# DeepBlender/DeepDenoiser

Hardware: AMD Instinct MI355X
Metric: train tiles/sec (128x128x32ch U-Net KPCN) (higher is better)
Workload: dtype bf16; 1 GPU; BASELINE config 2: U-Net [64,96,128]x4 + 5x5 KernelPrediction + 3-scale MultiScalePrediction, 32-channel render-pass stack, 128x128 tiles, full training step (fwd+SMAPE loss+bwd+Adam); global_batch=128, parallelism=dp1, hipgraph=True, inputs=resident in HBM

## Files before the change

deepdenoiser_amd/_lib.py:

```python

import ctypes as C
import os

_HERE = os.path.dirname(os.path.abspath(__file__))
LIB_PATH = os.environ.get("DD_LIB", os.path.join(_HERE, "libdd_hip.so"))

DD_F32, DD_BF16, DD_F16 = 0, 1, 2
IN_RELU, OUT_RELU, ACCUM, PIXSHUF, GATHER2X2 = 1, 2, 4, 8, 16
MAX_FEATURES, MAX_COMBINED = 32, 8
METRIC_SOURCES = MAX_FEATURES + MAX_COMBINED + 1
HISTOGRAM_DIFFERENCE, HISTOGRAM_VARIATION_DIFFERENCE, HISTOGRAM_MASKED_DIFFERENCE = 0, 1, 2
HISTOGRAM_VALUES_SCRATCH_BYTES = 20480
PREVIEW_SOURCE, PREVIEW_PREDICTION, PREVIEW_TARGET, PREVIEW_DIFFERENCE = 1, 2, 4, 8
PREVIEW_MAX_IMAGES, PREVIEW_THRESHOLDS = 16, 255
NONFINITE_MAX_PLANES = 32
QUALITY_MAX_PAIRS, QUALITY_TILE = 32, 32
GRAD_CHUNK, GRAD_PARTIAL_BYTES = 4096, 24


def histogram_stats_offset(nb):
    return (nb + 1) // 2 * 8


def histogram_record_bytes(nb):
    return histogram_stats_offset(nb) + 48


SYMBOLS = (
    "dd_version", "dd_last_error", "dd_pack_weights", "dd_pack_weights_batched", "dd_conv_igemm", "dd_conv_wgrad", "dd_colsum", "dd_colsum_segments",
    "dd_maxpool_fwd", "dd_maxpool_bwd", "dd_avgpool", "dd_prepare_feature", "dd_gather_input",
    "dd_kpcn_fwd", "dd_kpcn_bwd", "dd_kpcn_hidden_fwd", "dd_kpcn_hidden_bwd", "dd_compose_pack", "dd_compose_blend_fwd", "dd_compose_blend_bwd",
    "dd_compose_unpack_bwd", "dd_invert_std_fwd", "dd_invert_std_bwd", "dd_loss_head", "dd_adam_step",
    "dd_stitch", "dd_recombine", "dd_probe_tr16", "dd_masked_add", "dd_zero_stuff", "dd_zero_unstuff", "dd_convert_channels",
    "dd_augment", "dd_loss_mask_sums", "dd_crc32c", "dd_extract_tiles", "dd_compose_net_fwd", "dd_compose_net_bwd",
    "dd_kpcn_head_fwd", "dd_kpcn_head_bwd", "dd_kpcn_head_bwd_multi", "dd_assemble_input", "dd_assemble_input_frames", "dd_conv3x3_bwd", "dd_conv3x3_bwd_multi", "dd_convt2x2_fwd", "dd_convt2x2_bwd", "dd_convt_bwd_wide_count", "dd_conv3x3_ks",
    "dd_conv_pw_count", "dd_wgrad_pw_count", "dd_conv_route_count", "dd_space_to_depth2", "dd_convt3_wgrad", "dd_compose_stream_plan", "dd_compose_bwd_scratch_bytes",
    "dd_loss_msssim_scratch_bytes", "dd_loss_msssim_fwd", "dd_loss_msssim_bwd", "dd_loss_msssim_values",
    "dd_loss_metrics_scratch_bytes", "dd_loss_metrics", "dd_loss_head_path_count",
    "dd_loss_head_dscale", "dd_loss_msssim_bwd_dscale", "dd_grads_nonfinite", "dd_adam_step_scaled", "dd_scaler_update",
    "dd_histogram_values", "dd_loss_histograms_scratch_bytes", "dd_loss_histograms", "dd_loss_previews",
    "dd_nonfinite_scan", "dd_nonfinite_repair", "dd_frame_quality_scratch_bytes", "dd_frame_quality", "dd_stitch_blend",
    "dd_grad_norms", "dd_adam_step_clipped", "dd_adam_step_scaled_clipped", "dd_sample_tiles",
)


ROUTES = ("igemm_resident", "igemm_streamed", "igemm_ws", "rw_6_2", "rw12", "rw12_mask", "rw12_res", "rw8_kc2", "rw8_kc4", "rw8_kc4_mask", "pw",
          "ks", "ks_pw_taps", "wgrad_dma", "wgrad_reg", "wgrad_pw", "wgrad_stacked")


def route_counts():
    lib = load()
    return {name: lib.dd_conv_route_count(r) for r, name in enumerate(ROUTES)}


SUBROUTES = ("rw8_k32",)


def subroute_counts():
    lib = load()
    return {name: lib.dd_conv_route_count(len(ROUTES) + r) for r, name in enumerate(SUBROUTES)}


class ConvT3WgradArgs(C.Structure):
    _fields_ = [("s", C.c_void_p), ("lds", C.c_int), ("cout", C.c_int), ("cp", C.c_int),
                ("x", C.c_void_p), ("ldx", C.c_int), ("cin", C.c_int),
                ("dk", C.c_void_p),
                ("B", C.c_int), ("H", C.c_int), ("W", C.c_int), ("dtype", C.c_int)]


class ConvArgs(C.Structure):
    _fields_ = [("x", C.c_void_p), ("ldx", C.c_int), ("cin", C.c_int),
                ("wp", C.c_void_p), ("k_pad", C.c_int), ("n_pad", C.c_int),
                ("bias", C.c_void_p), ("nbias", C.c_int),
                ("res", C.c_void_p), ("ldres", C.c_int),
                ("mask", C.c_void_p), ("ldmask", C.c_int),
                ("y", C.c_void_p), ("ldy", C.c_int), ("n", C.c_int),
                ("B", C.c_int), ("H", C.c_int), ("W", C.c_int),
                ("taps", C.c_int), ("flags", C.c_int), ("dtype", C.c_int)]


class WgradArgs(C.Structure):
    _fields_ = [("p", C.c_void_p), ("ldp", C.c_int), ("m", C.c_int),
                ("q", C.c_void_p), ("ldq", C.c_int), ("n", C.c_int),
                ("out", C.c_void_p), ("bias_out", C.c_void_p), ("bias_mode", C.c_int),
                ("B", C.c_int), ("H", C.c_int), ("W", C.c_int),
                ("taps", C.c_int), ("flags", C.c_int), ("dtype", C.c_int), ("ksplit", C.c_int),
                ("stack_blocks", C.c_int), ("stack_width", C.c_int), ("stack_m0", C.c_int),
                ("stack_out", C.c_void_p * 8), ("stack_bias", C.c_void_p * 8)]
# ... 205 lines not shown
    if _lib is not None:
        return _lib
    import torch
    if not os.path.exists(LIB_PATH):
        raise RuntimeError("libdd_hip.so is not built (%s missing): run `python -m deepdenoiser_amd.build`. "
                           "There is no CPU/PyTorch fallback for the hot path." % LIB_PATH)
    lib = C.CDLL(LIB_PATH)
    missing = [s for s in SYMBOLS if not hasattr(lib, s)]
    if missing:
        raise RuntimeError("libdd_hip.so lacks symbols %s: rebuild it" % missing)
    lib.dd_version.restype = C.c_char_p
    lib.dd_last_error.restype = C.c_char_p
    _check_source_hash(lib)
    for s in SYMBOLS[2:]:
        getattr(lib, s).restype = C.c_int
    vp, i, l, f = C.c_void_p, C.c_int, C.c_long, C.c_float
    lib.dd_pack_weights.argtypes = [vp, vp, i, i, i, i, i, i, l, l, l, i, vp]
    lib.dd_pack_weights_batched.argtypes = [vp, i, i, vp]
    lib.dd_conv_igemm.argtypes = [C.POINTER(ConvArgs), vp]
    lib.dd_conv_wgrad.argtypes = [C.POINTER(WgradArgs), vp]
    lib.dd_conv3x3_bwd.argtypes = [C.POINTER(ConvBwdArgs), vp]
    lib.dd_conv3x3_bwd_multi.argtypes = [C.POINTER(ConvBwdArgs), i, vp]
    lib.dd_convt2x2_fwd.argtypes = [C.POINTER(ConvTArgs), vp]
    lib.dd_convt2x2_bwd.argtypes = [C.POINTER(ConvTArgs), vp]
    lib.dd_conv3x3_ks.argtypes = [C.POINTER(ConvKsArgs), vp]
    lib.dd_space_to_depth2.argtypes = [vp, i, vp, i, i, i, i, i, i, i, vp]
    lib.dd_convt3_wgrad.argtypes = [C.POINTER(ConvT3WgradArgs), vp]
    lib.dd_conv_pw_count.argtypes = []
    lib.dd_conv_pw_count.restype = C.c_long
    lib.dd_wgrad_pw_count.argtypes = []
    lib.dd_wgrad_pw_count.restype = C.c_long
    lib.dd_convt_bwd_wide_count.argtypes = []
    lib.dd_convt_bwd_wide_count.restype = C.c_long
    lib.dd_conv_route_count.argtypes = [i]
    lib.dd_conv_route_count.restype = C.c_long
    lib.dd_colsum.argtypes = [vp, i, i, l, vp, i, vp]
    lib.dd_colsum_segments.argtypes = [vp, i, i, l, i, vp, i, vp, i, vp]
    lib.dd_maxpool_fwd.argtypes = [vp, i, vp, i, vp, i, i, i, i, i, i, i, i, vp]
    lib.dd_maxpool_bwd.argtypes = [vp, i, vp, vp, i, vp, i, i, i, i, i, i, i, i, i, vp]
    lib.dd_avgpool.argtypes = [vp, i, vp, i, i, i, i, i, i, vp]
    lib.dd_prepare_feature.argtypes = [vp, i, vp, i, C.POINTER(FeatureParams), i, i, i, vp]
    lib.dd_gather_input.argtypes = [vp, i, i, vp, i, i, i, i, i, i, vp]
    lib.dd_kpcn_fwd.argtypes = [vp, i, vp, i, vp, i, i, i, i, i, i, vp]
    lib.dd_kpcn_bwd.argtypes = [vp, i, vp, i, vp, i, vp, i, i, i, i, i, i, i, vp]
    lib.dd_kpcn_hidden_fwd.argtypes = [vp, i, vp, i, i, vp, i, vp, vp, i, i, i, i, i, i, vp]
    lib.dd_kpcn_hidden_bwd.argtypes = [vp, i, vp, i, i, vp, i, vp, vp, i, vp, i, i, i, i, i, i, i, vp]
    lib.dd_compose_pack.argtypes = [vp, i, vp, i, vp, i, i, i, i, i, i, vp]
    lib.dd_compose_blend_fwd.argtypes = [vp, i, vp, i, vp, i, vp, i, i, i, i, i, vp]
    lib.dd_compose_blend_bwd.argtypes = [vp, i, vp, i, vp, i, vp, i, vp, i, i, vp, i, vp, i, i, i, i, i, i, vp]
    lib.dd_compose_unpack_bwd.argtypes = [vp, i, vp, i, vp, i, i, i, i, i, vp]
    lib.dd_invert_std_fwd.argtypes = [vp, vp, l, i, f, f, vp]
    lib.dd_invert_std_bwd.argtypes = [vp, vp, vp, l, i, f, f, vp]
    lib.dd_loss_head.argtypes = [C.POINTER(LossDesc), i, i, i, vp, f, vp]
    lib.dd_loss_head_path_count.argtypes = [i]
    lib.dd_loss_head_path_count.restype = C.c_long
    lib.dd_loss_msssim_scratch_bytes.argtypes = [i, i, i, i]
    lib.dd_loss_msssim_scratch_bytes.restype = C.c_long
    lib.dd_loss_msssim_fwd.argtypes = [C.POINTER(MsSsimDesc), i, i, i, vp, vp, vp]
    lib.dd_loss_msssim_bwd.argtypes = [C.POINTER(MsSsimDesc), i, i, i, vp, f, vp]
    lib.dd_loss_msssim_values.argtypes = [C.POINTER(MsSsimDesc), i, i, i, vp, vp, vp]
    lib.dd_loss_metrics_scratch_bytes.argtypes = [i, i, i]
    lib.dd_loss_metrics_scratch_bytes.restype = C.c_long
    lib.dd_loss_metrics.argtypes = [C.POINTER(LossDesc), i, i, i, vp, vp, vp]
    lib.dd_histogram_values.argtypes = [vp, l, vp, i, vp, vp, vp]
    lib.dd_loss_histograms_scratch_bytes.argtypes = [i, i, i, i]
    lib.dd_loss_histograms_scratch_bytes.restype = C.c_long
# ... 48 lines not shown
```

deepdenoiser_amd/csrc/dd_conv_bwd.hip:

```cpp
#include "dd_common.h"

#ifndef CBW_DF_RING
#define CBW_DF_RING 2
#endif
#ifndef CBW_REUSE
#define CBW_REUSE 1
#endif
#ifndef BW_DMA_SPAN
#define BW_DMA_SPAN 8
#endif
namespace {

struct BwdP {
  const void* dy; const void* x; const void* wd; void* dx; float* dw; float* db;
  int lddy, ldx, lddx;
  int cout, cin, coutv, cinv;
  int n_pad, k_pad;
  int B, H, W, tiles_x, tiles_y;
  int nblk, nblk_co, ksplit;
  int co_base;
  int use_mask, accumulate;
};

typedef __attribute__((address_space(3))) s16x4_t* lds_tr_ptr;
// ... 4 lines not shown

__device__ __forceinline__ void bw_dma_1k(const void* gptr, unsigned lds_addr) {
  asm volatile("s_mov_b32 m0, %1\n\ts_nop 0\n\tglobal_load_lds_dwordx4 %0, off" : : "v"(gptr), "s"(lds_addr) : "memory");
}

typedef uint32_t bw_u32x4 __attribute__((ext_vector_type(4)));
typedef uint32_t bw_u32x2 __attribute__((ext_vector_type(2)));
__device__ __forceinline__ uint4 bw_lds16(unsigned off) {
  const bw_u32x4 v = *reinterpret_cast<const __attribute__((address_space(3))) bw_u32x4*>(off);
  return uint4{v[0], v[1], v[2], v[3]};
}
__device__ __forceinline__ uint2 bw_lds8(unsigned off) {
  const bw_u32x2 v = *reinterpret_cast<const __attribute__((address_space(3))) bw_u32x2*>(off);
  return uint2{v[0], v[1]};
}
__device__ __forceinline__ uint4 bw_tr_pair(unsigned a0, unsigned a1) {
  const s16x4_t lo = __builtin_amdgcn_ds_read_tr16_b64_v4i16(reinterpret_cast<lds_tr_ptr>(a0));
  const s16x4_t hi = __builtin_amdgcn_ds_read_tr16_b64_v4i16(reinterpret_cast<lds_tr_ptr>(a1));
  const uint2 l2 = __builtin_bit_cast(uint2, lo), h2 = __builtin_bit_cast(uint2, hi);
  const uint4 v = {l2.x, l2.y, h2.x, h2.y};
  return v;
}

template <typename T> __device__ __forceinline__ void bw_mma_inplace(f32x4_t& acc, const uint4& a, const uint4& b);
template <> __device__ __forceinline__ void bw_mma_inplace<bf16_t>(f32x4_t& acc, const uint4& a, const uint4& b) {
  const bw_u32x4 av = {a.x, a.y, a.z, a.w}, bv = {b.x, b.y, b.z, b.w};
  asm volatile("v_mfma_f32_16x16x32_bf16 %0, %1, %2, %0" : "+v"(acc) : "v"(av), "v"(bv));
}
template <> __device__ __forceinline__ void bw_mma_inplace<f16_t>(f32x4_t& acc, const uint4& a, const uint4& b) {
  const bw_u32x4 av = {a.x, a.y, a.z, a.w}, bv = {b.x, b.y, b.z, b.w};
  asm volatile("v_mfma_f32_16x16x32_f16 %0, %1, %2, %0" : "+v"(acc) : "v"(av), "v"(bv));
}

template <typename T, bool MASK, bool ACCUM>
__device__ __forceinline__ void conv_bwd_body(const BwdP& a, char* smem, int block) {
  static_assert(sizeof(T) == 2, "fused conv backward: bf16 / fp16 storage");
  constexpr int PW = BW_PW;
  const int tid = threadIdx.x, lane = tid & 63, wave = __builtin_amdgcn_readfirstlane(tid >> 6);
  const int pair = block / a.ksplit, ks = block - pair * a.ksplit;
  const int cb = pair % a.nblk, ob = pair / a.nblk + (a.co_base >> 6);
  const int wr = wave & 3;
  const unsigned lds_base = (unsigned)(uintptr_t)(__attribute__((address_space(3))) char*)smem;
  const int per_img = a.tiles_y * a.tiles_x;
  const int total_tiles = a.B * per_img;
#ifdef CBW_EXP_NO_XCD
  const int xcd_n = 1;
#else
  const int xcd_n = (a.ksplit & 7) == 0 ? 8 : 1;
#endif
  const int per_xcd = a.ksplit / xcd_n;
  const int tile0 = (ks % xcd_n) * per_xcd + ks / xcd_n;

  if (wave < 4) {
    constexpr int QPC = 8, PPC = (BW_PCH + 3) / 4, NP = QPC + PPC;
    const T* __restrict__ DY = reinterpret_cast<const T*>(a.dy);
    const T* __restrict__ X = reinterpret_cast<const T*>(a.x);
    const int r = lane >> 3, ls = (lane & 7) ^ r;
    const int xch = cb * 64 + ls * 8, dch = ob * 64 + ls * 8;
    const bool x_ok = xch < a.cinv, d_ok = dch < a.coutv;
    const char* zero = reinterpret_cast<const char*>(&dd_zero16_v);
    const int x_row = a.W * a.ldx * 2, x_lane = (r * a.ldx + xch) * 2;
    const int dy_row = a.W * a.lddy * 2, dy_pix = a.lddy * 2, dy_lane = dch * 2;
    struct Origin { const char* q; const char* p; int b, y0, x0; bool live; };
    auto origin = [&](int tile) {
      Origin o;
      o.live = tile < total_tiles;
      const int t = o.live ? tile : 0;
// ... 119 lines not shown
          }
          if (j == 2 && yy >= 3) write_row(yy - 3);
          {
            constexpr int SPAN = NF * BW_DMA_SPAN / 8 > NP ? NF * BW_DMA_SPAN / 8 : NP;
            const int k0 = (f * NP + SPAN - 1) / SPAN;
            if (k0 < NP && (k0 * SPAN) / NP == f) piece(k0, on, sel ^ 1);
          }
          __builtin_amdgcn_sched_barrier(0);
#pragma unroll
          for (int dy = 0; dy < 3; ++dy) {
            const int y = yy - dy;
            if (y >= 0 && y < DD_TILE) acc[y % 4] = mma16<T>(wf[dy * 3 + dx][kc], ring[f % RING], acc[y % 4]);
          }
#ifndef CBW_EXP_ONE_BARRIER
          __builtin_amdgcn_sched_barrier(0);
#endif
        }
      }
      write_row(DD_TILE - 1);
      const int flip = sel ? -BW_BUF : BW_BUF;
#pragma unroll
      for (int c = 0; c < 8; ++c) d0[c] += flip;
      mrow += flip;
      oc = on;
    }
  } else {
    const int li = lane & 15, q4 = (lane >> 4) * 4;
#ifdef CBW_EXP_NO_WROLE
    const bool active = false;
#else
    const bool active = ob * 64 + wr * 16 < a.cout;
#endif
    const bool bias_wave = a.db != nullptr && cb == 0;
    const int nci = min(4, (a.cin - cb * 64 + 15) >> 4);
    unsigned pb[8], qb[2];
    {
      const int t16 = lane & 15, gq = lane >> 4, sub = t16 & 3;
      const int yl = gq >> 1, xl = (gq & 1) * 8 + (t16 >> 2), halfb = (sub & 1) * 8;
      const int pl = yl * PW + xl, ql = yl * DD_TILE + xl;
#pragma unroll
      for (int c = 0; c < 8; ++c) pb[c] = lds_base + pl * DD_LDS_ROW + (((wr * 2 + (sub >> 1)) ^ ((pl + c) & 7)) << 4) + halfb;
#pragma unroll
      for (int h = 0; h < 2; ++h)
        qb[h] = lds_base + BW_P_BYTES + ql * DD_LDS_ROW + (((sub >> 1) ^ ((ql + 4 * h) & 7)) << 4) + halfb;
    }
    f32x4_t acc[9][4];
#pragma unroll
    for (int t = 0; t < 9; ++t)
#pragma unroll
      for (int i = 0; i < 4; ++i) acc[t][i] = f32x4_t{0.f, 0.f, 0.f, 0.f};
    float bsum = 0.f;
    auto x_frag = [&](int s, int i) {
      return bw_tr_pair((qb[0] ^ (i << 5)) + (2 * s * DD_TILE) * DD_LDS_ROW, (qb[1] ^ (i << 5)) + (2 * s * DD_TILE + 4) * DD_LDS_ROW);
    };
    auto dy_frag = [&](int step) {
      const int s = step / 9, t = step - 9 * s;
      const int c0 = (2 * s + t / 3) * PW + t % 3;
      return bw_tr_pair(pb[c0 & 7] + c0 * DD_LDS_ROW, pb[(c0 + 4) & 7] + (c0 + 4) * DD_LDS_ROW);
    };

    int sel = 0;
    for (int tile = tile0; tile < total_tiles; tile += a.ksplit, sel ^= 1) {
      __syncthreads();
      if (!active) continue;
      constexpr int DFR = CBW_DF_RING, DFA = DFR - 1;
      uint4 xf[2][4], df[DFR];
#if CBW_REUSE
      uint4 keep[3];
#define CBW_NEEDS_READ(st) (!((st) >= 9 && (st) % 9 < 3))
#else
#define CBW_NEEDS_READ(st) true
#endif
#pragma unroll
      for (int i = 0; i < 4; ++i) xf[0][i] = x_frag(0, i);
#pragma unroll
      for (int n = 0; n < DFA; ++n) df[n] = dy_frag(n);
#pragma unroll
      for (int s = 0; s < 8; ++s)
#pragma unroll
      for (int t = 0; t < 9; ++t) {
        const int step = s * 9 + t;
        if (step + DFA < 72 && CBW_NEEDS_READ(step + DFA)) df[(step + DFA) % DFR] = dy_frag(step + DFA);
#ifdef CBW_EXP_HALF_X
        if (s + 1 < 8 && t >= 4 && t < 6) xf[(s + 1) & 1][t - 4] = x_frag(s + 1, t - 4);
#else
        if (s + 1 < 8 && t >= 4 && t < 8) xf[(s + 1) & 1][t - 4] = x_frag(s + 1, t - 4);
#endif
        __builtin_amdgcn_sched_barrier(0);
#if CBW_REUSE
        const uint4 cur = (s > 0 && t < 3) ? keep[t] : df[step % DFR];
        if (t >= 6) keep[t - 6] = cur;
#else
        const uint4 cur = df[step % DFR];
#endif
#ifdef CBW_EXP_HALF_MMA
#pragma unroll
        for (int i = 0; i < 2; ++i) bw_mma_inplace<T>(acc[t][i], xf[s & 1][i], cur);
#else
#pragma unroll
        for (int i = 0; i < 4; ++i) bw_mma_inplace<T>(acc[t][i], xf[s & 1][i], cur);
#endif
        if (t == 4 && bias_wave) {
          float f[8];
          unpack8t<T>(df[step % DFR], f);
          bsum += ((f[0] + f[1]) + (f[2] + f[3])) + ((f[4] + f[5]) + (f[6] + f[7]));
        }
#ifndef CBW_EXP_ONE_BARRIER_W
        __builtin_amdgcn_sched_barrier(0);
#endif
      }
      const int flip = sel ? -BW_BUF : BW_BUF;
#pragma unroll
      for (int c = 0; c < 8; ++c) pb[c] += flip;
      qb[0] += flip; qb[1] += flip;
    }

    asm volatile("s_nop 15\n\ts_nop 15" ::: "memory");
    dd_det_wait();
    if (active) {
      const int co = ob * 64 + wr * 16 + li;
      if (co < a.cout) {
#pragma unroll
        for (int t = 0; t < 9; ++t)
#pragma unroll
          for (int i = 0; i < 4; ++i) {
            if (i >= nci) continue;
#pragma unroll
            for (int e = 0; e < 4; ++e) {
              const int ci = cb * 64 + i * 16 + q4 + e;
#ifdef CBW_EXP_NO_FLUSH
              if (ci < a.cin && acc[t][i][e] == 123.456f) atomicAdd(a.dw + ((long)(8 - t) * a.cin + ci) * a.cout + co, acc[t][i][e]);
#else
              if (ci < a.cin) atomicAdd(a.dw + ((long)(8 - t) * a.cin + ci) * a.cout + co, acc[t][i][e]);
#endif
            }
          }
      }
      if (bias_wave) {
        float b = bsum;
        b += __shfl_xor(b, 16);
        b += __shfl_xor(b, 32);
        if (lane < 16 && co < a.cout) atomicAdd(a.db + co, b);
      }
    }
  }
  dd_det_end();
}

template <typename T, bool MASK, bool ACCUM>
__global__ __launch_bounds__(512) void conv_bwd_kernel(const BwdP a) {
  extern __shared__ __attribute__((aligned(1024))) char smem[];
  conv_bwd_body<T, MASK, ACCUM>(a, smem, blockIdx.x);
}

constexpr int BW_MAX_MULTI = 4;
struct BwdMulti { BwdP p[BW_MAX_MULTI]; int blocks[BW_MAX_MULTI]; };
template <typename T>
__global__ __launch_bounds__(512) void conv_bwd_multi_kernel(const BwdMulti m) {
  extern __shared__ __attribute__((aligned(1024))) char smem[];
  if ((int)blockIdx.x >= m.blocks[blockIdx.y]) {
    dd_det_wait();
    dd_det_end();
    return;
  }
  conv_bwd_body<T, false, false>(m.p[blockIdx.y], smem, blockIdx.x);
}

static int bwd_cus() {
  return dd_device_cus();
}

template <typename T, bool MASK, bool ACCUM>
int launch_bwd_flags(const BwdP& p, hipStream_t stream) {
  const size_t lds = 2 * (size_t)BW_BUF;
  dd_det_sync();
  dd_allow_max_lds(reinterpret_cast<const void*>(conv_bwd_kernel<T, MASK, ACCUM>));
  const long blocks = (long)p.nblk * p.nblk_co * p.ksplit;
  hipLaunchKernelGGL((conv_bwd_kernel<T, MASK, ACCUM>), dim3((unsigned)blocks), dim3(512), lds, stream, p);
  DD_LAUNCH_CHECK();
  return DD_OK;
}
template <typename T>
int launch_bwd(const BwdP& p, hipStream_t stream) {
  if (p.use_mask) return p.accumulate ? launch_bwd_flags<T, true, true>(p, stream) : launch_bwd_flags<T, true, false>(p, stream);
  return p.accumulate ? launch_bwd_flags<T, false, true>(p, stream) : launch_bwd_flags<T, false, false>(p, stream);
}

}

static int bwd_fill(BwdP& p, const dd_conv_bwd_args* a);
int dd_conv_bwd96_launch(const dd_conv_bwd_args* a, hipStream_t stream);

extern "C" int dd_conv3x3_bwd_multi(const dd_conv_bwd_args* a, int n, dd_stream stream) {
  DD_REQUIRE(a && n >= 1 && n <= BW_MAX_MULTI, "dd_conv3x3_bwd_multi: 1 to %d problems", BW_MAX_MULTI);
  BwdMulti m;
  memset(&m, 0, sizeof(m));
  long gx = 1;
  for (int i = 0; i < n; ++i) {
    DD_REQUIRE(a[i].dx == nullptr && a[i].B == a[0].B && a[i].H == a[0].H && a[i].W == a[0].W && a[i].dtype == a[0].dtype && !a[i].use_mask && !a[i].accumulate,
               "dd_conv3x3_bwd_multi: problem %d: weight-gradient-only problems (dx = NULL) on one [B, H, W] grid and storage type", i);
    if (int rc = bwd_fill(m.p[i], &a[i])) return rc;
    BwdP& p = m.p[i];
    const long total_tiles = (long)p.B * p.tiles_x * p.tiles_y;
    p.nblk_co = dd_ceil_div(p.cout, 64);
    long ksplit = bwd_cus() / ((long)n * p.nblk * p.nblk_co);
    if (ksplit < 1) ksplit = 1;
    if (ksplit > total_tiles) ksplit = total_tiles;
    p.ksplit = (int)ksplit; p.co_base = 0; p.use_mask = 0; p.accumulate = 0;
    m.blocks[i] = p.nblk * p.nblk_co * p.ksplit;
    if (m.blocks[i] > gx) gx = m.blocks[i];
  }
  hipStream_t s = reinterpret_cast<hipStream_t>(stream);
  const size_t lds = 2 * (size_t)BW_BUF;
  dd_det_sync();
  if (a[0].dtype == DD_BF16) {
    dd_allow_max_lds(reinterpret_cast<const void*>(conv_bwd_multi_kernel<bf16_t>));
    hipLaunchKernelGGL(conv_bwd_multi_kernel<bf16_t>, dim3((unsigned)gx, (unsigned)n), dim3(512), lds, s, m);
  } else {
    dd_allow_max_lds(reinterpret_cast<const void*>(conv_bwd_multi_kernel<f16_t>));
    hipLaunchKernelGGL(conv_bwd_multi_kernel<f16_t>, dim3((unsigned)gx, (unsigned)n), dim3(512), lds, s, m);
  }
  DD_LAUNCH_CHECK();
// ... 6 lines not shown
  DD_REQUIRE(a->cout > 0 && a->cin > 0, "dd_conv3x3_bwd: cout=%d cin=%d", a->cout, a->cin);
  const int coutv = (a->cout + 7) / 8 * 8, cinv = (a->cin + 7) / 8 * 8;
  DD_REQUIRE(a->ld_dy % 8 == 0 && a->ld_x % 8 == 0 && coutv <= a->ld_dy && cinv <= a->ld_x && (!a->dx || (a->ld_dx % 4 == 0 && cinv <= a->ld_dx)),
             "dd_conv3x3_bwd: ld_dy=%d ld_x=%d ld_dx=%d must cover the channel counts rounded to 8 (ld_dy, ld_x multiples of 8)", a->ld_dy, a->ld_x, a->ld_dx);
  DD_REQUIRE(((uintptr_t)a->dy % 16) == 0 && ((uintptr_t)a->x % 16) == 0 && ((uintptr_t)a->wd % 16) == 0 && ((uintptr_t)a->dx % 8) == 0,
             "dd_conv3x3_bwd: dy / x / wd must be 16-byte aligned, dx 8-byte aligned");
  DD_REQUIRE(!a->dx || (a->n_pad >= a->cin && a->k_pad >= a->cout && a->k_pad % 8 == 0), "dd_conv3x3_bwd: packed weights [9][n_pad=%d][k_pad=%d] do not cover %d x %d", a->n_pad, a->k_pad, a->cin, a->cout);
  DD_REQUIRE(a->B > 0 && a->H > 0 && a->W > 0 && (long)a->B * a->H * a->W < (1L << 31) / 256, "dd_conv3x3_bwd: empty or oversized grid");
  p.dy = a->dy; p.x = a->x; p.wd = a->wd; p.dx = a->dx; p.dw = a->dw; p.db = a->db;
  p.lddy = a->ld_dy; p.ldx = a->ld_x; p.lddx = a->ld_dx;
  p.cout = a->cout; p.cin = a->cin; p.coutv = coutv; p.cinv = cinv;
  p.n_pad = a->n_pad; p.k_pad = a->k_pad;
  p.B = a->B; p.H = a->H; p.W = a->W;
  p.tiles_x = dd_ceil_div(a->W, DD_TILE); p.tiles_y = dd_ceil_div(a->H, DD_TILE);
  p.nblk = dd_ceil_div(a->cin, 64);
  p.nblk_co = 1; p.ksplit = 1; p.co_base = 0; p.use_mask = a->use_mask; p.accumulate = a->accumulate;
  return DD_OK;
}

extern "C" int dd_conv3x3_bwd(const dd_conv_bwd_args* a, dd_stream stream) {
  BwdP p;
  if (int rc = bwd_fill(p, a)) return rc;
  const long total_tiles = (long)a->B * p.tiles_x * p.tiles_y;
  hipStream_t s = reinterpret_cast<hipStream_t>(stream);
  static const bool bwd96 = [] { const char* e = getenv("DD_CONV_BWD96"); return !(e && e[0] == '0'); }();
  if (bwd96 && a->dx && a->cout > 64 && a->cout <= 96) return dd_conv_bwd96_launch(a, s);
  const int n_launch = a->dx ? dd_ceil_div(a->cout, 64) : 1;
  p.nblk_co = a->dx ? 1 : dd_ceil_div(a->cout, 64);
  long ksplit = bwd_cus() / (p.nblk * p.nblk_co);
  if (ksplit < 1) ksplit = 1;
  if (ksplit > total_tiles) ksplit = total_tiles;
  p.ksplit = (int)ksplit;
  p.use_mask = a->use_mask;
  for (int l = 0; l < n_launch; ++l) {
    p.co_base = l * 64;
    p.accumulate = a->accumulate || l > 0;
    const int rc = a->dtype == DD_BF16 ? launch_bwd<bf16_t>(p, s) : launch_bwd<f16_t>(p, s);
    if (rc != DD_OK) return rc;
  }
  return DD_OK;
}
```

deepdenoiser_amd/csrc/dd_conv_rw.hip:

```cpp
#include "dd_common.h"

namespace {

struct RwP {
  const void* x; const void* wp; const float* bias; const void* mask; void* y;
  int ldx, ldmask, ldy;
  int cin, cinv, n, n_pad, k_pad, nbias;
  int B, H, W, tiles_x, tiles_y, nblk, ksplit;
  int relu, accum, aux_residual;
};

typedef uint32_t rw_u32x4 __attribute__((ext_vector_type(4)));
typedef uint32_t rw_u32x2 __attribute__((ext_vector_type(2)));
constexpr int RW_TW = 16, RW_TH = 8, RW_PW = RW_TW + 2, RW_PH = RW_TH + 2;
constexpr int RW_CH = (RW_PW * RW_PH + 7) / 8;
constexpr int RW_SLICE = RW_CH * 1024, RW_BUF = 2 * RW_SLICE;

__device__ __forceinline__ void rw_dma_1k(const void* gptr, unsigned lds_addr) {
  asm volatile("s_mov_b32 m0, %1\n\ts_nop 0\n\tglobal_load_lds_dwordx4 %0, off" : : "v"(gptr), "s"(lds_addr) : "memory");
}
__device__ __forceinline__ uint4 rw_lds16(unsigned off) {
  const rw_u32x4 v = *reinterpret_cast<const __attribute__((address_space(3))) rw_u32x4*>(off);
  return uint4{v[0], v[1], v[2], v[3]};
}
// ... 281 lines not shown
  }
  float bv[4];
#pragma unroll
  for (int e = 0; e < 4; ++e) bv[e] = (AUX != 1 && a.bias && active && c4 + e < a.nbias) ? a.bias[c4 + e] : 0.f;
  unsigned m_off = 0;
  if (MASKED) {
    const int c4l = (wave % CT) * 16 + q * 4, rr = li & 7;
    m_off = mask_base + ((c4l >> 6) * MCH + half * RH * 2 + (li >> 3)) * 1024 + rr * 128 + (((((c4l & 63) >> 3)) ^ rr) << 4) + ((c4l >> 2) & 1) * 8;
  }
  unsigned d0[8];
#pragma unroll
  for (int c = 0; c < 8; ++c) d0[c] = lds_base + (half * RH * PW + li) * DD_LDS_ROW + ((q ^ ((half * RH * PW + li + c) & 7)) << 4);
  T* __restrict__ Y = reinterpret_cast<T*>(a.y);
  const bool ch_ok = active && c4 < a.n;
  const long yrow = (long)a.W * a.ldy;

  int sel = 0;
  for (int tile = tile0; tile < total; tile += a.ksplit, sel ^= 1) {
    __builtin_amdgcn_s_waitcnt(0x0F70);
    __syncthreads();
    const RwTile nxt = tile_at(tile + a.ksplit);
    const unsigned nbuf = lds_base + (sel ^ 1) * G::BUF, nmbuf = mask_base + (sel ^ 1) * MBUF;
    if (!active) {
#pragma unroll
      for (int k = 0; k < NPIECE; ++k) piece(k, nxt, nbuf);
#pragma unroll
      for (int k = 0; k < NMP; ++k) mpiece(k, nxt, nmbuf);
      cur = nxt;
      continue;
    }
    const bool col_ok = ch_ok && cur.x0 + li < a.W;
    T* yp = Y + (((long)cur.b * a.H + cur.y0 + half * RH) * a.W + cur.x0 + li) * a.ldy + c4;
    f32x4_t acc[4];
    constexpr int FR = 3 * KC, NF = PHW * FR, RING = NW == 8 ? 6 : 2, AHEAD = RING - 1;
    rw_u32x4 ring[RING], r0 = {0u, 0u, 0u, 0u}, r1 = r0;
    auto slot = [&](int i) -> rw_u32x4& { if constexpr (RING == 2) return (i & 1) ? r1 : r0; else return ring[i % RING]; };
    auto frag = [&](int f) {
      const int yy = f / FR, j = f - FR * yy, dx = j / KC, kc = j - KC * dx, C = yy * PW + dx;
      return *reinterpret_cast<const __attribute__((address_space(3))) rw_u32x4*>((d0[C & 7] ^ ((kc & 1) << 6)) + (kc >> 1) * G::SLICE + C * DD_LDS_ROW);
    };
    uint2 mv = uint2{0u, 0u};
    auto read_mask = [&](int y) {
      const rw_u32x2 m = *reinterpret_cast<const __attribute__((address_space(3))) rw_u32x2*>(m_off + y * 2048);
      mv = uint2{m[0], m[1]};
    };
    auto write_row = [&](int y) {
      f32x4_t v = acc[y % 4];
      uint2 o2;
      o2.x = pack2<T>(v[0], v[1]);
      o2.y = pack2<T>(v[2], v[3]);
      if (AUX == 1) { o2.x = mask_bf16x2_cmp(o2.x, mv.x); o2.y = mask_bf16x2_cmp(o2.y, mv.y); }
      if (AUX == 2) {
        float f8[8], g8[8];
        unpack8t<T>(uint4{o2.x, o2.y, 0u, 0u}, f8);
        unpack8t<T>(uint4{mv.x, mv.y, 0u, 0u}, g8);
        o2.x = pack2<T>(f8[0] + g8[0], f8[1] + g8[1]);
        o2.y = pack2<T>(f8[2] + g8[2], f8[3] + g8[3]);
      }
      if (AUX != 1 && a.relu) { o2.x = relu_bf16x2(o2.x); o2.y = relu_bf16x2(o2.y); }
#ifdef RW_EXP_NO_STORE
      if (col_ok && cur.y0 + half * RH + y < a.H && o2.x == 0x12345678u) *reinterpret_cast<uint2*>(yp + y * yrow) = o2;
#else
      if (col_ok && cur.y0 + half * RH + y < a.H) *reinterpret_cast<uint2*>(yp + y * yrow) = o2;
#endif
    };
#pragma unroll
    for (int f = 0; f < AHEAD; ++f) slot(f) = frag(f);
// ... 80 lines not shown
  static int on8m = -1;
  if (on8m < 0) { const char* e = getenv("DD_CONV_RW8_MASK"); on8m = e ? atoi(e) : 1; }
  const bool wide = a->cin > 96 && a->cin <= 128 && a->k_pad <= 128;
  const bool mask_ok = !a->mask || (on8m && wide && !a->res && !a->bias && !(a->flags & DD_OUT_RELU) && a->n % 8 == 0 && a->ldmask % 8 == 0 && ((uintptr_t)a->mask % 16) == 0);
  return on8 && ((a->cin > 16 && a->cin <= 64 && a->k_pad <= 64) || wide) && mask_ok && !(a->flags & DD_ACCUM) && a->n >= 48;
}

template <typename T, int KC, int NW = 8, int AUX = 0>
static void rw8_launch(const RwP& p, hipStream_t stream) {
  constexpr size_t mask_lds = AUX ? 2 * (size_t)((NW / 2 * 16 + 63) / 64) * (DD_TILE * RfGeo<KC>::TH / 8) * 1024 : 0;
  static_assert(2 * (size_t)RfGeo<KC>::BUF + mask_lds <= 160 * 1024, "LDS");
  dd_allow_max_lds(reinterpret_cast<const void*>(conv_rw8_kernel<T, KC, NW, AUX>));
  hipLaunchKernelGGL((conv_rw8_kernel<T, KC, NW, AUX>), dim3((unsigned)(p.nblk * p.ksplit)), dim3(NW * 64), 2 * (size_t)RfGeo<KC>::BUF + mask_lds, stream, p);
}

int dd_conv_rw_launch(const dd_conv_args* a, hipStream_t stream) {
  RwP p;
  p.x = a->x; p.wp = a->wp; p.bias = a->bias; p.mask = a->res ? a->res : a->mask; p.y = a->y;
  p.ldx = a->ldx; p.ldmask = a->res ? a->ldres : a->ldmask; p.ldy = a->ldy; p.aux_residual = a->res != nullptr;
  p.cin = a->cin; p.cinv = (a->cin + 7) / 8 * 8; p.n = a->n; p.n_pad = a->n_pad; p.k_pad = a->k_pad; p.nbias = a->nbias;
  p.B = a->B; p.H = a->H; p.W = a->W;
  p.relu = (a->flags & DD_OUT_RELU) != 0; p.accum = (a->flags & DD_ACCUM) != 0;
  static int on12 = -1;
  if (on12 < 0) { const char* e = getenv("DD_CONV_RW12"); on12 = e ? atoi(e) : 1; }
  const bool plain_fwd = !a->mask && !a->res && !(a->flags & DD_ACCUM);
  static int on12m = -1;
  if (on12m < 0) { const char* e = getenv("DD_CONV_RW12_MASK"); on12m = e ? atoi(e) : 1; }
  const bool masked12 = on12 && on12m && a->cin > 64 && a->cin <= 96 && a->mask && !a->res && !a->bias && !(a->flags & (DD_ACCUM | DD_OUT_RELU)) &&
                        a->n >= 48 && a->n % 8 == 0 && a->ldmask % 8 == 0 && ((uintptr_t)a->mask % 16) == 0;
  const bool res12 = on12 && on12m && a->cin > 64 && a->cin <= 96 && a->res && !a->mask && !(a->flags & DD_ACCUM) && a->n >= 48 && a->n % 8 == 0 &&
                     a->ldres % 8 == 0 && ((uintptr_t)a->res % 16) == 0;
  const bool twelve = on12 && a->cin > 64 && a->cin <= 96 && (plain_fwd || masked12 || res12) && a->n >= 48;
  const bool six = a->cin > 64 && a->cin <= 96 && !twelve;
  const int th = six ? RW_TH : (a->cin <= 64 ? RfGeo<2>::TH : RfGeo<4>::TH);
  p.tiles_x = dd_ceil_div(a->W, DD_TILE); p.tiles_y = dd_ceil_div(a->H, th);
  p.nblk = dd_ceil_div(a->n, (six || twelve) ? 96 : 64);
  const long total = (long)a->B * p.tiles_x * p.tiles_y;
  long ksplit = rw_cus() / p.nblk;
  if (ksplit < 1) ksplit = 1;
  if (ksplit > total) ksplit = total;
  p.ksplit = (int)ksplit;
  if (masked12) {
    DD_ROUTE_TAKEN(DD_ROUTE_RW12_MASK);
    if (a->dtype == DD_BF16) rw8_launch<bf16_t, 3, 12, 1>(p, stream); else rw8_launch<f16_t, 3, 12, 1>(p, stream);
  } else if (res12) {
    DD_ROUTE_TAKEN(DD_ROUTE_RW12_RES);
    if (a->dtype == DD_BF16) rw8_launch<bf16_t, 3, 12, 2>(p, stream); else rw8_launch<f16_t, 3, 12, 2>(p, stream);
  } else if (twelve) {
    DD_ROUTE_TAKEN(DD_ROUTE_RW12);
    if (a->dtype == DD_BF16) rw8_launch<bf16_t, 3, 12>(p, stream); else rw8_launch<f16_t, 3, 12>(p, stream);
  } else if (six) {
    DD_ROUTE_TAKEN(DD_ROUTE_RW_6_2);
    if (a->dtype == DD_BF16) rw_launch_flags<bf16_t, 3>(p, stream); else rw_launch_flags<f16_t, 3>(p, stream);
  } else if (a->cin <= 64) {
    static int on_k32 = -1;
    if (on_k32 < 0) { const char* e = getenv("DD_CONV_RW8_K32"); on_k32 = e ? atoi(e) : 1; }
    static_assert(RfGeo<1>::TH == RfGeo<2>::TH && RfGeo<1>::BUF == RfGeo<2>::BUF, "one K chunk: the tiles of KC = 2");
    DD_ROUTE_TAKEN(DD_ROUTE_RW8_KC2);
    if (on_k32 && a->cin <= 32 && a->k_pad == 32) {
      DD_ROUTE_TAKEN(DD_ROUTE_RW8_K32);
      if (a->dtype == DD_BF16) rw8_launch<bf16_t, 1>(p, stream); else rw8_launch<f16_t, 1>(p, stream);
    } else if (a->dtype == DD_BF16) rw8_launch<bf16_t, 2>(p, stream); else rw8_launch<f16_t, 2>(p, stream);
  } else if (a->mask) {
    DD_ROUTE_TAKEN(DD_ROUTE_RW8_KC4_MASK);
    if (a->dtype == DD_BF16) rw8_launch<bf16_t, 4, 8, 1>(p, stream); else rw8_launch<f16_t, 4, 8, 1>(p, stream);
  } else {
    DD_ROUTE_TAKEN(DD_ROUTE_RW8_KC4);
    if (a->dtype == DD_BF16) rw8_launch<bf16_t, 4>(p, stream); else rw8_launch<f16_t, 4>(p, stream);
  }
  DD_LAUNCH_CHECK();
  return DD_OK;
}
```

include/dd_hip.h:

```cpp
#ifndef DD_HIP_H
#define DD_HIP_H

#include <stddef.h>
#include <stdint.h>

#ifdef __cplusplus
extern "C" {
#endif

typedef void* dd_stream;

enum dd_dtype { DD_F32 = 0, DD_BF16 = 1, DD_F16 = 2 };

enum dd_status {
  DD_OK = 0,
  DD_ERR_INVALID = -1,
  DD_ERR_LAUNCH = -2
};

enum dd_conv_flags {
  DD_IN_RELU = 1,
  DD_OUT_RELU = 2,
  DD_ACCUM = 4,
  DD_PIXSHUF = 8,
// ... 11 lines not shown

typedef struct {
  const void* x; int ldx; int cin;
  const void* wp; int k_pad; int n_pad;
  const float* bias; int nbias;
  const void* res; int ldres;
  const void* mask; int ldmask;
  void* y; int ldy; int n;
  int B, H, W;
  int taps; int flags; int dtype;
} dd_conv_args;
int dd_conv_igemm(const dd_conv_args* a, dd_stream stream);
long dd_conv_pw_count(void);
long dd_wgrad_pw_count(void);
enum dd_conv_route {
  DD_ROUTE_IGEMM_RESIDENT = 0,
  DD_ROUTE_IGEMM_STREAMED,
  DD_ROUTE_IGEMM_WS,
  DD_ROUTE_RW_6_2,
  DD_ROUTE_RW12,
  DD_ROUTE_RW12_MASK,
  DD_ROUTE_RW12_RES,
  DD_ROUTE_RW8_KC2,
  DD_ROUTE_RW8_KC4,
  DD_ROUTE_RW8_KC4_MASK,
  DD_ROUTE_PW,
  DD_ROUTE_KS,
  DD_ROUTE_KS_PW_TAPS,
  DD_ROUTE_WGRAD_DMA,
  DD_ROUTE_WGRAD_REG,
  DD_ROUTE_WGRAD_PW,
  DD_ROUTE_WGRAD_STACKED,
  DD_ROUTE_RW8_K32,
  DD_ROUTE_COUNT
};
long dd_conv_route_count(int route);

typedef struct {
  const void* p; int ldp; int m;
  const void* q; int ldq; int n;
  float* out;
  float* bias_out; int bias_mode;
  int B, H, W;
  int taps; int flags; int dtype;
  int ksplit;
  int stack_blocks; int stack_width; int stack_m0;
  float* stack_out[8]; float* stack_bias[8];
} dd_wgrad_args;
int dd_conv_wgrad(const dd_wgrad_args* a, dd_stream stream);

typedef struct {
  const void* dy; int ld_dy; int cout;
  const void* x; int ld_x; int cin;
  const void* wd; int n_pad; int k_pad;
  void* dx; int ld_dx;
  float* dw; float* db;
  int B, H, W;
  int use_mask; int accumulate; int dtype;
} dd_conv_bwd_args;
int dd_conv3x3_bwd(const dd_conv_bwd_args* a, dd_stream stream);
int dd_conv3x3_bwd_multi(const dd_conv_bwd_args* a, int n, dd_stream stream);

typedef struct {
  const void* x; int ld_x; int cin;
  void* y; int ld_y; int cout;
  const void* w; int n_pad; int k_pad;
  const float* bias; int relu;
  void* dx; int ld_dx; float* dw; float* db; int use_mask; int accumulate;
  int B, H, W;
  int dtype;
} dd_convt_args;
int dd_convt2x2_fwd(const dd_convt_args* a, dd_stream stream);
int dd_convt2x2_bwd(const dd_convt_args* a, dd_stream stream);
long dd_convt_bwd_wide_count(void);

typedef struct {
  const void* x; int ldx; int cin;
  const void* wp; int n_pad; int k_pad;
  const float* bias; int nbias;
  void* y; int ldy;
  int n0; int n;
  int B, H, W;
  int mode; int flags; int dtype;
  const void* mask; int ldmask;
} dd_conv_ks_args;
int dd_conv3x3_ks(const dd_conv_ks_args* a, dd_stream stream);

int dd_colsum(const void* x, int ld, int c, long rows, float* out, int dtype, dd_stream stream);
int dd_colsum_segments(const void* x, int ld, int c, long rows_per_segment, int n_segments, float* out, int out_ld, const int* out_row,
                       int dtype, dd_stream stream);

int dd_maxpool_fwd(const void* x, int ldx, void* y, int ldy, uint8_t* idx, int C, int B, int H, int W,
                   int pool, int stride, int relu_mask, int dtype, dd_stream stream);
// ... 293 lines not shown
```

Before: 16210 tiles/s.

## Add shape-specialized conv routes: NCI=2 wgrad backward, 96-wide K64 and 64-wide K96 forward tiles

Adds an NCI template parameter to the fused conv backward kernel so that weight-gradient-only launches with cin<=32 use a two-fragment variant. This variant has a smaller accumulator array and runs in a single launch. In the forward register-window path, cin 33-64 layers with output width 65-96 get a 12-wave, 96-column route, and KC<=2 kernels get a deeper fragment ring. cin 65-96 layers whose output width pads less at 64 than at 96 get an 8-wave, 64-column tile. All routes default on behind env toggles, and the aim is to cut wasted padded columns and register pressure, at the risk of lower occupancy or worse scheduling on the new instantiations.

```diff
diff --git a/deepdenoiser_amd/_lib.py b/deepdenoiser_amd/_lib.py
--- a/deepdenoiser_amd/_lib.py
+++ b/deepdenoiser_amd/_lib.py
@@ -33,7 +33,7 @@
     "dd_compose_unpack_bwd", "dd_invert_std_fwd", "dd_invert_std_bwd", "dd_loss_head", "dd_adam_step",
     "dd_stitch", "dd_recombine", "dd_probe_tr16", "dd_masked_add", "dd_zero_stuff", "dd_zero_unstuff", "dd_convert_channels",
     "dd_augment", "dd_loss_mask_sums", "dd_crc32c", "dd_extract_tiles", "dd_compose_net_fwd", "dd_compose_net_bwd",
-    "dd_kpcn_head_fwd", "dd_kpcn_head_bwd", "dd_kpcn_head_bwd_multi", "dd_assemble_input", "dd_assemble_input_frames", "dd_conv3x3_bwd", "dd_conv3x3_bwd_multi", "dd_convt2x2_fwd", "dd_convt2x2_bwd", "dd_convt_bwd_wide_count", "dd_conv3x3_ks",
+    "dd_kpcn_head_fwd", "dd_kpcn_head_bwd", "dd_kpcn_head_bwd_multi", "dd_assemble_input", "dd_assemble_input_frames", "dd_conv3x3_bwd", "dd_conv3x3_bwd_multi", "dd_convt2x2_fwd", "dd_convt2x2_bwd", "dd_convt_bwd_wide_count", "dd_conv_bwd_nci2_count", "dd_conv3x3_ks",
     "dd_conv_pw_count", "dd_wgrad_pw_count", "dd_conv_route_count", "dd_space_to_depth2", "dd_convt3_wgrad", "dd_compose_stream_plan", "dd_compose_bwd_scratch_bytes",
     "dd_loss_msssim_scratch_bytes", "dd_loss_msssim_fwd", "dd_loss_msssim_bwd", "dd_loss_msssim_values",
     "dd_loss_metrics_scratch_bytes", "dd_loss_metrics", "dd_loss_head_path_count",
@@ -53,7 +53,7 @@
     return {name: lib.dd_conv_route_count(r) for r, name in enumerate(ROUTES)}
 
 
-SUBROUTES = ("rw8_k32",)
+SUBROUTES = ("rw8_k32", "rw12_k64", "rw8_k96")
 
 
 def subroute_counts():
@@ -325,6 +325,8 @@
     lib.dd_wgrad_pw_count.restype = C.c_long
     lib.dd_convt_bwd_wide_count.argtypes = []
     lib.dd_convt_bwd_wide_count.restype = C.c_long
+    lib.dd_conv_bwd_nci2_count.argtypes = []
+    lib.dd_conv_bwd_nci2_count.restype = C.c_long
     lib.dd_conv_route_count.argtypes = [i]
     lib.dd_conv_route_count.restype = C.c_long
     lib.dd_colsum.argtypes = [vp, i, i, l, vp, i, vp]
diff --git a/deepdenoiser_amd/csrc/dd_conv_bwd.hip b/deepdenoiser_amd/csrc/dd_conv_bwd.hip
--- a/deepdenoiser_amd/csrc/dd_conv_bwd.hip
+++ b/deepdenoiser_amd/csrc/dd_conv_bwd.hip
@@ -60,7 +60,7 @@
   asm volatile("v_mfma_f32_16x16x32_f16 %0, %1, %2, %0" : "+v"(acc) : "v"(av), "v"(bv));
 }
 
-template <typename T, bool MASK, bool ACCUM>
+template <typename T, bool MASK, bool ACCUM, int NCI = 4>
 __device__ __forceinline__ void conv_bwd_body(const BwdP& a, char* smem, int block) {
   static_assert(sizeof(T) == 2, "fused conv backward: bf16 / fp16 storage");
   constexpr int PW = BW_PW;
@@ -246,7 +246,7 @@
     const bool active = ob * 64 + wr * 16 < a.cout;
 #endif
     const bool bias_wave = a.db != nullptr && cb == 0;
-    const int nci = min(4, (a.cin - cb * 64 + 15) >> 4);
+    const int nci = min(NCI, (a.cin - cb * 64 + 15) >> 4);
     unsigned pb[8], qb[2];
     {
       const int t16 = lane & 15, gq = lane >> 4, sub = t16 & 3;
@@ -258,11 +258,11 @@
       for (int h = 0; h < 2; ++h)
         qb[h] = lds_base + BW_P_BYTES + ql * DD_LDS_ROW + (((sub >> 1) ^ ((ql + 4 * h) & 7)) << 4) + halfb;
     }
-    f32x4_t acc[9][4];
+    f32x4_t acc[9][NCI];
 #pragma unroll
     for (int t = 0; t < 9; ++t)
 #pragma unroll
-      for (int i = 0; i < 4; ++i) acc[t][i] = f32x4_t{0.f, 0.f, 0.f, 0.f};
+      for (int i = 0; i < NCI; ++i) acc[t][i] = f32x4_t{0.f, 0.f, 0.f, 0.f};
     float bsum = 0.f;
     auto x_frag = [&](int s, int i) {
       return bw_tr_pair((qb[0] ^ (i << 5)) + (2 * s * DD_TILE) * DD_LDS_ROW, (qb[1] ^ (i << 5)) + (2 * s * DD_TILE + 4) * DD_LDS_ROW);
@@ -278,7 +278,7 @@
       __syncthreads();
       if (!active) continue;
       constexpr int DFR = CBW_DF_RING, DFA = DFR - 1;
-      uint4 xf[2][4], df[DFR];
+      uint4 xf[2][NCI], df[DFR];
 #if CBW_REUSE
       uint4 keep[3];
 #define CBW_NEEDS_READ(st) (!((st) >= 9 && (st) % 9 < 3))
@@ -286,7 +286,7 @@
 #define CBW_NEEDS_READ(st) true
 #endif
 #pragma unroll
-      for (int i = 0; i < 4; ++i) xf[0][i] = x_frag(0, i);
+      for (int i = 0; i < NCI; ++i) xf[0][i] = x_frag(0, i);
 #pragma unroll
       for (int n = 0; n < DFA; ++n) df[n] = dy_frag(n);
 #pragma unroll
@@ -298,7 +298,7 @@
 #ifdef CBW_EXP_HALF_X
         if (s + 1 < 8 && t >= 4 && t < 6) xf[(s + 1) & 1][t - 4] = x_frag(s + 1, t - 4);
 #else
-        if (s + 1 < 8 && t >= 4 && t < 8) xf[(s + 1) & 1][t - 4] = x_frag(s + 1, t - 4);
+        if (s + 1 < 8 && t >= 4 && t < 4 + NCI) xf[(s + 1) & 1][t - 4] = x_frag(s + 1, t - 4);
 #endif
         __builtin_amdgcn_sched_barrier(0);
 #if CBW_REUSE
@@ -312,7 +312,7 @@
         for (int i = 0; i < 2; ++i) bw_mma_inplace<T>(acc[t][i], xf[s & 1][i], cur);
 #else
 #pragma unroll
-        for (int i = 0; i < 4; ++i) bw_mma_inplace<T>(acc[t][i], xf[s & 1][i], cur);
+        for (int i = 0; i < NCI; ++i) bw_mma_inplace<T>(acc[t][i], xf[s & 1][i], cur);
 #endif
         if (t == 4 && bias_wave) {
           float f[8];
@@ -337,7 +337,7 @@
 #pragma unroll
         for (int t = 0; t < 9; ++t)
 #pragma unroll
-          for (int i = 0; i < 4; ++i) {
+          for (int i = 0; i < NCI; ++i) {
             if (i >= nci) continue;
 #pragma unroll
             for (int e = 0; e < 4; ++e) {
@@ -361,10 +361,10 @@
   dd_det_end();
 }
 
-template <typename T, bool MASK, bool ACCUM>
+template <typename T, bool MASK, bool ACCUM, int NCI = 4>
 __global__ __launch_bounds__(512) void conv_bwd_kernel(const BwdP a) {
   extern __shared__ __attribute__((aligned(1024))) char smem[];
-  conv_bwd_body<T, MASK, ACCUM>(a, smem, blockIdx.x);
+  conv_bwd_body<T, MASK, ACCUM, NCI>(a, smem, blockIdx.x);
 }
 
 constexpr int BW_MAX_MULTI = 4;
@@ -384,13 +384,13 @@
   return dd_device_cus();
 }
 
-template <typename T, bool MASK, bool ACCUM>
+template <typename T, bool MASK, bool ACCUM, int NCI = 4>
 int launch_bwd_flags(const BwdP& p, hipStream_t stream) {
   const size_t lds = 2 * (size_t)BW_BUF;
   dd_det_sync();
-  dd_allow_max_lds(reinterpret_cast<const void*>(conv_bwd_kernel<T, MASK, ACCUM>));
+  dd_allow_max_lds(reinterpret_cast<const void*>(conv_bwd_kernel<T, MASK, ACCUM, NCI>));
   const long blocks = (long)p.nblk * p.nblk_co * p.ksplit;
-  hipLaunchKernelGGL((conv_bwd_kernel<T, MASK, ACCUM>), dim3((unsigned)blocks), dim3(512), lds, stream, p);
+  hipLaunchKernelGGL((conv_bwd_kernel<T, MASK, ACCUM, NCI>), dim3((unsigned)blocks), dim3(512), lds, stream, p);
   DD_LAUNCH_CHECK();
   return DD_OK;
 }
@@ -402,6 +402,7 @@
 
 }
 
+static long bwd_nci2_launches = 0;
 static int bwd_fill(BwdP& p, const dd_conv_bwd_args* a);
 int dd_conv_bwd96_launch(const dd_conv_bwd_args* a, hipStream_t stream);
 
@@ -474,6 +475,12 @@
   if (ksplit > total_tiles) ksplit = total_tiles;
   p.ksplit = (int)ksplit;
   p.use_mask = a->use_mask;
+  static const bool nci2 = [] { const char* e = getenv("DD_CONV_BWD_NCI2"); return !(e && e[0] == '0'); }();
+  if (nci2 && !a->dx && a->cin <= 32) {
+    p.co_base = 0; p.use_mask = 0; p.accumulate = 0;
+    ++bwd_nci2_launches;
+    return a->dtype == DD_BF16 ? launch_bwd_flags<bf16_t, false, false, 2>(p, s) : launch_bwd_flags<f16_t, false, false, 2>(p, s);
+  }
   for (int l = 0; l < n_launch; ++l) {
     p.co_base = l * 64;
     p.accumulate = a->accumulate || l > 0;
@@ -482,3 +489,5 @@
   }
   return DD_OK;
 }
+
+extern "C" long dd_conv_bwd_nci2_count(void) { return bwd_nci2_launches; }
diff --git a/deepdenoiser_amd/csrc/dd_conv_rw.hip b/deepdenoiser_amd/csrc/dd_conv_rw.hip
--- a/deepdenoiser_amd/csrc/dd_conv_rw.hip
+++ b/deepdenoiser_amd/csrc/dd_conv_rw.hip
@@ -337,7 +337,7 @@
     const bool col_ok = ch_ok && cur.x0 + li < a.W;
     T* yp = Y + (((long)cur.b * a.H + cur.y0 + half * RH) * a.W + cur.x0 + li) * a.ldy + c4;
     f32x4_t acc[4];
-    constexpr int FR = 3 * KC, NF = PHW * FR, RING = NW == 8 ? 6 : 2, AHEAD = RING - 1;
+    constexpr int FR = 3 * KC, NF = PHW * FR, RING = (NW == 8 || KC <= 2) ? 6 : 2, AHEAD = RING - 1;
     rw_u32x4 ring[RING], r0 = {0u, 0u, 0u, 0u}, r1 = r0;
     auto slot = [&](int i) -> rw_u32x4& { if constexpr (RING == 2) return (i & 1) ? r1 : r0; else return ring[i % RING]; };
     auto frag = [&](int f) {
@@ -484,9 +484,14 @@
                      a->ldres % 8 == 0 && ((uintptr_t)a->res % 16) == 0;
   const bool twelve = on12 && a->cin > 64 && a->cin <= 96 && (plain_fwd || masked12 || res12) && a->n >= 48;
   const bool six = a->cin > 64 && a->cin <= 96 && !twelve;
+  static int on_k64 = -1, on_k96 = -1;
+  if (on_k64 < 0) { const char* e = getenv("DD_CONV_RW12_K64"); on_k64 = e ? atoi(e) : 1; }
+  if (on_k96 < 0) { const char* e = getenv("DD_CONV_RW8_K96"); on_k96 = e ? atoi(e) : 1; }
+  const bool k64_12 = on_k64 && plain_fwd && a->cin > 32 && a->cin <= 64 && a->n > 64 && a->n <= 96;
+  const bool k96_8 = on_k96 && twelve && plain_fwd && dd_ceil_div(a->n, 64) * 64 - a->n < dd_ceil_div(a->n, 96) * 96 - a->n;
   const int th = six ? RW_TH : (a->cin <= 64 ? RfGeo<2>::TH : RfGeo<4>::TH);
   p.tiles_x = dd_ceil_div(a->W, DD_TILE); p.tiles_y = dd_ceil_div(a->H, th);
-  p.nblk = dd_ceil_div(a->n, (six || twelve) ? 96 : 64);
+  p.nblk = dd_ceil_div(a->n, ((six || twelve) && !k96_8) || k64_12 ? 96 : 64);
   const long total = (long)a->B * p.tiles_x * p.tiles_y;
   long ksplit = rw_cus() / p.nblk;
   if (ksplit < 1) ksplit = 1;
@@ -500,7 +505,10 @@
     if (a->dtype == DD_BF16) rw8_launch<bf16_t, 3, 12, 2>(p, stream); else rw8_launch<f16_t, 3, 12, 2>(p, stream);
   } else if (twelve) {
     DD_ROUTE_TAKEN(DD_ROUTE_RW12);
-    if (a->dtype == DD_BF16) rw8_launch<bf16_t, 3, 12>(p, stream); else rw8_launch<f16_t, 3, 12>(p, stream);
+    if (k96_8) {
+      DD_ROUTE_TAKEN(DD_ROUTE_RW8_K96);
+      if (a->dtype == DD_BF16) rw8_launch<bf16_t, 3, 8>(p, stream); else rw8_launch<f16_t, 3, 8>(p, stream);
+    } else if (a->dtype == DD_BF16) rw8_launch<bf16_t, 3, 12>(p, stream); else rw8_launch<f16_t, 3, 12>(p, stream);
   } else if (six) {
     DD_ROUTE_TAKEN(DD_ROUTE_RW_6_2);
     if (a->dtype == DD_BF16) rw_launch_flags<bf16_t, 3>(p, stream); else rw_launch_flags<f16_t, 3>(p, stream);
@@ -512,6 +520,9 @@
     if (on_k32 && a->cin <= 32 && a->k_pad == 32) {
       DD_ROUTE_TAKEN(DD_ROUTE_RW8_K32);
       if (a->dtype == DD_BF16) rw8_launch<bf16_t, 1>(p, stream); else rw8_launch<f16_t, 1>(p, stream);
+    } else if (k64_12) {
+      DD_ROUTE_TAKEN(DD_ROUTE_RW12_K64);
+      if (a->dtype == DD_BF16) rw8_launch<bf16_t, 2, 12>(p, stream); else rw8_launch<f16_t, 2, 12>(p, stream);
     } else if (a->dtype == DD_BF16) rw8_launch<bf16_t, 2>(p, stream); else rw8_launch<f16_t, 2>(p, stream);
   } else if (a->mask) {
     DD_ROUTE_TAKEN(DD_ROUTE_RW8_KC4_MASK);
diff --git a/include/dd_hip.h b/include/dd_hip.h
--- a/include/dd_hip.h
+++ b/include/dd_hip.h
@@ -67,6 +67,8 @@
   DD_ROUTE_WGRAD_PW,
   DD_ROUTE_WGRAD_STACKED,
   DD_ROUTE_RW8_K32,
+  DD_ROUTE_RW12_K64,
+  DD_ROUTE_RW8_K96,
   DD_ROUTE_COUNT
 };
 long dd_conv_route_count(int route);
@@ -94,6 +96,7 @@
   int use_mask; int accumulate; int dtype;
 } dd_conv_bwd_args;
 int dd_conv3x3_bwd(const dd_conv_bwd_args* a, dd_stream stream);
+long dd_conv_bwd_nci2_count(void);
 int dd_conv3x3_bwd_multi(const dd_conv_bwd_args* a, int n, dd_stream stream);
 
 typedef struct {
```

Result: slower. 16040 tiles/s (-1.0%).
